# will-rowe/groot

Hardware: AMD Instinct MI355X
Metric: Mreads/s aligned (higher is better)
Workload: dtype u64

## Files before the change

### groot_amd/csrc/hip/device_types.hpp

```cpp
#pragma once

#include <cstdint>

#include <hip/hip_runtime.h>

#include "groot_hip.h"

namespace groot {

constexpr int kBlock = 256;
constexpr uint32_t kEmpty = 0xFFFFFFFFu;

enum : uint32_t {
    kFlagShortRead = 1u,
    kFlagLongRead = 2u,
    kFlagSeedOverflow = 4u,
    kFlagTravOverflow = 8u,
    kFlagOrdOverflow = 16u,
    kFlagOvfOverflow = 32u,
    kFlagQOverflow = 64u,
};

constexpr uint32_t kIncrCap = 8;
constexpr uint32_t kIncrCapBig = 2048;
// ... 167 lines not shown

struct AlignArgs {
    DeviceIndex ix;
    const uint8_t *seq;
    const uint64_t *seq_off;
    uint32_t n_reads, first_read_id;
    uint32_t seed_slots;
    const uint32_t *seed_count;
    const uint32_t *seed_win;
    const uint32_t *perm;
    const ReadRec *read_rec;
    uint32_t no_align, update_weights;
    const void *node_rec;
    uint32_t *attempts;
    groot_trav *trav_first;
    uint64_t *mask_first;
    uint32_t *trav_cnt;
    groot_trav *ovf_trav;
    uint64_t *ovf_mask;
    uint32_t *ovf_cnt;
    uint32_t ovf_cap;
    uint64_t *stk_hdr;
    uint64_t *stk_mask;
    uint32_t n_threads, stk_depth;
    uint32_t lds_stride_dw;
    uint32_t *incr_cnt, *incr_win;
    uint32_t incr_cap;
    uint32_t head_lanes;
    uint32_t round_lanes;
    const uint4 *vitem;
    const uint32_t *vcount;
    uint32_t vcap;
    const uint32_t *n_perm;
    uint32_t refill;
    DeviceCounters *ctr;
};

struct alignas(16) LeanNode {
    uint32_t seq_off;
    uint32_t seq_len;
    uint32_t deg_kids;
    uint32_t pad;
    uint32_t edges[4];
    uint64_t first32;
    uint64_t mask[3];
};
static_assert(sizeof(LeanNode) == 64, "lean node record is one 64-byte line");
constexpr uint32_t kLeanNo = 0x80000000u;
struct alignas(16) LeanExt {
    uint64_t b[7];
    uint64_t pad;
};
static_assert(sizeof(LeanExt) == 64, "lean node extension is one 64-byte line");
constexpr uint32_t kLeanMaxLen = 256;

struct LeanArgs {
    const LeanNode *nodes;
    const LeanExt *ext;
    const uint32_t *bases2;
    const uint4 *cn_pre2;
    const uint64_t *node_l2b;
    const uint8_t *win_ok;
    const WinRec *win_rec;
    const uint32_t *q_row;
    const uint8_t *seq;
    const uint4 *packed;
    uint32_t packed_q;
    const uint32_t *perm;
    const ReadRec *read_rec;
    uint32_t n_reads, first_read_id, n_windows, k;
    uint32_t update_weights;
    uint32_t lds_stride_dw;
    uint32_t max_len;
    uint32_t *attempts;
    groot_trav *trav_first;
    uint64_t *mask_first;
    uint32_t *trav_cnt;
    uint8_t *defer;
    uint4 *stk;
    groot_trav *ovf_trav;
    uint64_t *ovf_mask;
    uint32_t *ovf_cnt;
    uint32_t ovf_cap;
    DeviceCounters *ctr;
    const uint4 *path_node;
    const uint32_t *path_text;
    const uint32_t *path_tag;
    const uint32_t *path_nodes;
    const uint64_t *path_tab;
    uint4 *hold;
};

__host__ __device__ inline uint32_t lean_stride_dw(uint32_t max_len) { return (((max_len + 15u) >> 4) + 15u) | 1u; }

}
```

### groot_amd/csrc/hip/groot_hip.hip

```cpp
#include <cstring>

#include <hip/hip_runtime.h>
#include <rocprim/rocprim.hpp>

#include <dlfcn.h>

#include <algorithm>
#include <cmath>
#include <cstdarg>
#include <cstdio>
#include <atomic>
#include <chrono>
#include <deque>
#include <map>
#include <memory>
#include <numeric>
#include <string>
#include <thread>
#include <vector>

#include "../common/cpus.hpp"
#include "../common/view_check.hpp"
#include "kernels_boot.hpp"
#include "kernels_cov.hpp"
// ... 94 lines not shown
    DevBuf<uint8_t> d_seq, d_exc_byte;
    DevBuf<uint64_t> d_off, d_exc_pos;
    uint32_t trav_cap = 0;
    DevBuf<groot_trav> d_trav;
    DevBuf<uint64_t> d_mask;
    DevBuf<DeviceCounters> d_ctr;
    PinBuf<DeviceCounters> h_ctr;
    PinBuf<groot_trav> h_trav;
    DevBuf<groot_ctrav> d_ctrav;
    PinBuf<groot_ctrav> h_ctrav;
    PinBuf<uint8_t> h_mask;
    PinBuf<uint32_t> h_ckpt;
    DevBuf<uint8_t> d_cmask;
    DevBuf<uint32_t> d_mwords, d_moff, d_ckpt;
    uint32_t n_trav = 0, copied = 0;
    uint64_t n_mask_bytes = 0, copied_bytes = 0;
    bool host_results = false;
    hipEvent_t ev_seed = nullptr;
    hipEvent_t ev_walk = nullptr;
    hipEvent_t ev_h2d0 = nullptr, ev_h2d = nullptr, ev_compute = nullptr, ev_ctr = nullptr, ev_d2h0 = nullptr, ev_d2h = nullptr;
    hipEvent_t ev[14]{};
    groot_counts counts{};
    int status = GROOT_OK;
    std::string status_msg;
    groot_stage_ms ms{};
    DevBuf<uint32_t> d_ec_slow;
    PinBuf<uint32_t> h_ec;
    const uint8_t *seq() const { return input == IN_DEVICE ? ext_seq : d_seq.p; }
    const uint64_t *off() const { return input == IN_DEVICE ? ext_off : d_off.p; }
};

struct WorkSet {
    DevBuf<uint32_t> seed_count, seed_win, perm, perm_count, trav_cnt, tab_idx;
    DevBuf<uint32_t> perm2, perm2_count;
    DevBuf<uint8_t> defer;
    DevBuf<uint4> packed;
    DevBuf<ReadRec> read_rec;
    DevBuf<uint4> vitem, split_list;
    DevBuf<uint32_t> vcount;
    DevBuf<groot_trav> trav_first;
    DevBuf<uint64_t> mask_first, sketches;
    DevBuf<groot_trav> ovf_trav;
    DevBuf<uint64_t> ovf_mask;
    DevBuf<uint32_t> ovf_cnt;
    hipEvent_t ev_free = nullptr;
    bool used = false;
    Slot *owner = nullptr;
    uint64_t ticket = 0;
};

struct groot_ctx {
    int device = 0;
    std::string err;
    groot_params prm{};
    Knobs kn;
    uint32_t s = 0, k = 0, max_k = 0, l_max = 0, pw_view = 0, pw = 0, n_windows = 0, max_q = 0, band_hash_bits = 0;
    hipEvent_t h2d_last = nullptr;
    Slot *newest = nullptr;
    hipEvent_t last_compute = nullptr;
    hipStream_t own_stream = nullptr, stream = nullptr, astream = nullptr, tstream = nullptr, own_tstream = nullptr, h2d_stream = nullptr, d2h_stream = nullptr;
    bool profiling = false;

    DevBuf<uint32_t> graph_win_end;
    DevBuf<uint4> cn_pre;
    DevBuf<uint64_t> node_l2b;
    DevBuf<uint32_t> win_prefix, edges, win_graph, cn_node,
        band_keys, band_ids;
    DevBuf<ExactEntry> band_hash;
// ... 47 lines not shown
    DeviceIndex *build_dix = nullptr;
    hipStream_t build_stream = nullptr;
    unsigned long long *build_shards = nullptr;

    std::vector<std::unique_ptr<Slot>> slots;
    std::deque<Slot *> inflight;
    uint64_t next_ticket = 1;
    Slot *waited = nullptr;
    double todo_frac = 1.0;
    double lean_left_frac = 1.0;
    uint32_t n_cu = 256;
    double dfs_frac = 1.0;
    double trav_per_read = 1.25;
    double bytes_per_trav = 0;
    bool packed_travs = false;
    std::vector<uint32_t> h_node_graph;
    DevBuf<uint8_t> graph_words;
    std::vector<uint8_t> h_graph_words;
    WorkSet ws[2];
    uint32_t next_set = 0;

    uint32_t seed_slots = 0;
    DevBuf<uint32_t> sort_key, sort_key_out, perm_in, todo_list, todo_count;
    DevBuf<uint32_t> long_list, long_count;
    uint32_t vcap = 0;
    uint32_t lsh_defer_rows = 0, lsh_cap = 0;
    DevBuf<unsigned long long> seed_shards;
    DevBuf<uint32_t> lsh_list, lsh_count;
    DevBuf<uint64_t> lsh_sketch;
    DevBuf<char> sort_tmp, in_tmp;
    uint32_t ovf_cap = 0;
    DevBuf<uint32_t> trav_off;
    DevBuf<char> scan_tmp;
    DevBuf<char> sel_tmp;
    uint32_t align_threads = 0, stk_depth = 0;
    DevBuf<uint64_t> stk_hdr, stk_mask;
    DevBuf<uint32_t> attempts, q_row, q_seen, q_of_row, q_nrows;
    uint32_t *attempts_ptr = nullptr;
    uint32_t att_cap = 0;
    bool att_external = false;
    bool cov_on = false;
    std::vector<uint32_t> h_cov_np_off, h_cov_gpo, h_cov_len;
    std::vector<uint2> h_cov_np;
    std::vector<uint64_t> h_cov_base;
    DevBuf<uint32_t> cov_np_off, cov_gpo, cov_len;
    DevBuf<uint2> cov_np;
    DevBuf<uint64_t> cov_base;
    DevBuf<unsigned long long> cov_starts, cov_ends;
    bool sh_on = false;
    uint32_t sh_tab_cap = 0;
    DevBuf<uint32_t> sh_gpo, sh_set_graph, sh_tab_rep, sh_tab_cnt, sh_slow, sh_batch;
    DevBuf<uint64_t> sh_set_mask;
    DevBuf<unsigned long long> sh_tri, sh_stats;
    bool ec_on = false;
    uint32_t ec_cap = 0, ec_epoch = 0;
    DevBuf<uint32_t> ec_claim, ec_graph, ec_fill;
    DevBuf<uint64_t> ec_mask;
    DevBuf<unsigned long long> ec_cnt;
    uint64_t ec_fill_known = 0;
    uint64_t ec_grows = 0, ec_slow_reads = 0;
    std::map<std::vector<uint32_t>, uint64_t> ec_host;
};

__attribute__((constructor)) static void groot_hw_queues() { setenv("GPU_MAX_HW_QUEUES", "8", 0); }

static thread_local std::string g_open_err;

// ... 253 lines not shown
static int grow_attempts(groot_ctx *c, uint32_t rows)
{
    if (c->att_external) return fail(c, GROOT_E_NOSPACE, "a kmerCount outside the fixed layout of groot_hip_attempts_layout occurred");
    DevBuf<uint32_t> bigger;
    HIP_TRY(c, bigger.alloc((size_t)rows * c->n_windows));
    HIP_TRY(c, hipMemset(bigger.p, 0, (size_t)rows * c->n_windows * sizeof(uint32_t)));
    if (c->attempts.p && c->att_cap)
        HIP_TRY(c, hipMemcpy(bigger.p, c->attempts.p, (size_t)std::min(rows, c->att_cap) * c->n_windows * sizeof(uint32_t), hipMemcpyDeviceToDevice));
    std::swap(c->attempts.p, bigger.p);
    std::swap(c->attempts.n, bigger.n);
    c->attempts_ptr = c->attempts.p;
    c->att_cap = rows;
    return GROOT_OK;
}

constexpr double kSparseBelow = 0.05;
struct HasKey {
    const uint32_t *key;
    __host__ __device__ bool operator()(uint32_t r) const { return key[r] != kEmpty; }
};
#ifndef GROOT_SPAN_BITS
#define GROOT_SPAN_BITS 6
#endif
static uint32_t list_lds_stride(uint32_t stride_dw)
{
    return kLdsReads + (uint64_t)kBlock * stride_dw * 4 <= 32 * 1024 ? stride_dw : 0;
}
#ifndef GROOT_HEAVY_BLOCKS
#define GROOT_HEAVY_BLOCKS 16384u
#endif
#ifndef GROOT_SORTLIST_BLOCKS
#define GROOT_SORTLIST_BLOCKS 16384
#endif
static int launch_seed_stage(groot_ctx *c, Slot *s, bool update_weights)
{
    WorkSet *w = &c->ws[s->set];
    SeedArgs a{};
    s->packed_q = 0;
    a.ix = c->dix;
    a.seq = s->seq();
    a.seq_off = s->off();
    a.n_reads = s->n_reads;
    a.max_read_len = c->prm.max_read_len;
    const uint64_t want = (uint64_t)kBlock * s->max_len + 32;
    a.lds_read_bytes = (uint32_t)std::min<uint64_t>(want, kMaxLdsReadBytes);
    a.seed_slots = c->seed_slots;
    a.seed_count = w->seed_count.p;
    a.seed_win = w->seed_win.p;
    a.sketch_out = c->prm.keep_sketches ? w->sketches.p : nullptr;
    a.sort_key = c->sort_key.p;
    a.read_rec = w->read_rec.p;
    a.q_seen = c->q_seen.p;
    a.trav_cnt = w->trav_cnt.p;
    a.shards = c->seed_shards.p;
    a.ctr = s->d_ctr.p;
    a.long_list = c->long_list.p; a.long_count = c->long_count.p;
    if (c->dix.out_tab) {
        a.tab_idx = w->tab_idx.p;
        a.tab_hist = c->tab_hist.p;
    }
    unsigned win_bits = 2;
    for (uint32_t v = c->n_windows ? c->n_windows - 1 : 0; v; v >>= 1) win_bits++;
    win_bits = std::min(32u, std::max(3u, win_bits));
    a.sort_span_bits = std::min((unsigned)GROOT_SPAN_BITS, 32u - win_bits);
    if (win_bits - 2u + a.sort_span_bits > 24u && win_bits - 2u + 4u <= 24u) a.sort_span_bits = 24u - (win_bits - 2u);
    a.sort_span_shift = win_bits;
// ... 58 lines not shown
    HIP_TRY(c, hipGetLastError());
    if (c->profiling) HIP_TRY(c, hipEventRecord(s->ev[12], c->stream));
    {
        SplitArgs sa{};
        sa.list = c->long_list.p; sa.count = c->long_count.p; sa.seed_count = w->seed_count.p; sa.seed_win = w->seed_win.p;
        sa.n_reads = s->n_reads; sa.seed_slots = c->seed_slots; sa.read_rec = w->read_rec.p; sa.win_rec = c->dix.win_rec;
        sa.split = c->vcap && !c->tab_capture && !c->prm.no_exact_align;
        sa.vitem = w->vitem.p; sa.vcount = w->vcount.p; sa.vcap = c->vcap; sa.split_list = w->split_list.p;
        sa.ctr = s->d_ctr.p; sa.update_weights = update_weights ? 1 : 0;
        hipLaunchKernelGGL(sort_seed_lists_kernel, dim3(GROOT_SORTLIST_BLOCKS), dim3(kBlock), 0, c->stream, sa);
    }
    if (c->profiling) HIP_TRY(c, hipEventRecord(s->ev[2], c->stream));
    hipLaunchKernelGGL(assign_q_rows_kernel, dim3(1), dim3(64), 0, c->stream, c->q_seen.p, c->q_row.p, c->q_of_row.p, c->q_nrows.p, c->att_cap,
                       c->max_q, s->d_ctr.p, c->seed_shards.p, c->long_count.p);
    if (a.tab_hist) {
        hipLaunchKernelGGL(fold_tab_hist_kernel, dim3(std::min<uint32_t>((c->n_windows + kBlock - 1) / kBlock, 1024u)), dim3(kBlock), 0, c->stream, c->tab_hist.p,
                           c->attempts_ptr, c->q_row.p, c->dix.w - c->k + 1, c->n_windows, s->d_ctr.p, update_weights ? 1u : 0u);
        HIP_TRY(c, hipGetLastError());
    }
    if (list_mode && a.dfs_list) return GROOT_OK;
    if (list_mode) {
        size_t tb = 0;
        HasKey pred{c->sort_key.p};
        rocprim::counting_iterator<uint32_t> ids(0u);
        HIP_TRY(c, rocprim::select(nullptr, tb, ids, w->perm.p, w->perm_count.p, (size_t)s->n_reads, pred, c->stream));
        if (tb > c->sort_tmp.n) {
            HIP_TRY(c, hipStreamSynchronize(c->stream));
            HIP_TRY(c, c->sort_tmp.alloc(tb + tb / 4));
        }
        HIP_TRY(c, rocprim::select(c->sort_tmp.p, tb, ids, w->perm.p, w->perm_count.p, (size_t)s->n_reads, pred, c->stream));
        return GROOT_OK;
    }
    size_t tmp_bytes = 0;
    HIP_TRY(c, rocprim::radix_sort_pairs(nullptr, tmp_bytes, c->sort_key.p, c->sort_key_out.p, c->perm_in.p, w->perm.p, s->n_reads, begin_bit,
                                         end_bit, c->stream));
    if (tmp_bytes > c->sort_tmp.n) {
        HIP_TRY(c, hipStreamSynchronize(c->stream));
        HIP_TRY(c, c->sort_tmp.alloc(tmp_bytes + tmp_bytes / 4));
    }
    HIP_TRY(c, rocprim::radix_sort_pairs(c->sort_tmp.p, tmp_bytes, c->sort_key.p, c->sort_key_out.p, c->perm_in.p, w->perm.p,
                                         s->n_reads, begin_bit, end_bit, c->stream));
    return GROOT_OK;
}

struct LeanLeft {
    const uint8_t *defer;
    const DeviceCounters *ctr;
    uint32_t lean_slots;
    __device__ uint8_t operator()(uint32_t i) const { return i < ctr->seeded_reads && (i >= lean_slots || defer[i]) ? 1 : 0; }
};

static int launch_align_stage(groot_ctx *c, Slot *s, bool update_weights)
{
    WorkSet *w = &c->ws[s->set];
    AlignArgs a{};
    a.ix = c->dix;
    a.seq = s->seq();
    a.seq_off = s->off();
    a.n_reads = s->n_reads;
    a.first_read_id = s->first_read_id;
    a.seed_slots = c->seed_slots;
    a.seed_count = w->seed_count.p;
    a.seed_win = w->seed_win.p;
    a.perm = w->perm.p;
    a.read_rec = w->read_rec.p;
    a.no_align = c->prm.no_exact_align;
    a.update_weights = update_weights ? 1 : 0;
    a.attempts = c->attempts_ptr;
    a.node_rec = c->node_rec.p;
    a.trav_first = w->trav_first.p;
    a.mask_first = w->mask_first.p;
    a.trav_cnt = w->trav_cnt.p;
    a.ovf_trav = w->ovf_trav.p;
    a.ovf_mask = w->ovf_mask.p;
    a.ovf_cnt = w->ovf_cnt.p;
    a.ovf_cap = c->ovf_cap;
    if (c->vcap) { a.vitem = w->vitem.p; a.vcount = w->vcount.p; a.vcap = c->vcap; }
    a.stk_hdr = c->stk_hdr.p;
    a.stk_mask = c->stk_mask.p;
    uint32_t blocks = std::min<uint32_t>((s->n_reads + kBlock - 1) / kBlock, c->align_threads / kBlock);
    if (c->dfs_frac < kSparseBelow && c->dfs_frac * (double)s->n_reads < 16.0 * (double)(blocks * (kBlock / 64))) blocks = std::max(1u, blocks / 2);
    else if (c->dfs_frac >= kSparseBelow && c->dfs_frac < 0.6 && !s->mixed_len && blocks >= 4) blocks /= 2;
    if ((s->lean_used || s->path_used) && c->lean_left_frac < 0.25) {
        uint32_t want = (uint32_t)(c->lean_left_frac * 1.25 * (double)s->n_reads / 64.0 / (kBlock / 64)) + 1u;
        blocks = std::max(1u, std::min(blocks, std::max(want, c->n_cu)));
    }
    a.n_threads = blocks * kBlock;
    a.stk_depth = c->stk_depth;
    {
        const uint32_t stride = (2 + 4 * ((s->max_len + 27) / 16)) | 1u;
        a.lds_stride_dw = (size_t)kBlock * stride * 4 <= 64 * 1024 ? stride : 0;
    }
    if (c->tab_capture) {
        a.incr_cnt = c->incr_cnt.p; a.incr_win = c->incr_win.p; a.incr_cap = c->incr_cap;
        HIP_TRY(c, hipMemsetAsync(c->incr_cnt.p, 0, (size_t)s->n_reads * sizeof(uint32_t), c->tstream));
    }
    a.head_lanes = s->mixed_len ? 16u : 0u;
#ifndef GROOT_REFILL_ERR
#define GROOT_REFILL_ERR 48
#endif
#ifndef GROOT_REFILL_MIXED
#define GROOT_REFILL_MIXED 2
#endif
    a.refill = s->mixed_len ? (uint32_t)GROOT_REFILL_MIXED : (c->dfs_frac >= kSparseBelow && c->dfs_frac < 0.6 ? (uint32_t)GROOT_REFILL_ERR : 64u);
#ifdef GROOT_WORK_COUNTERS
    if (const char *e = getenv("GROOT_DEV_ROUND")) a.round_lanes = (uint32_t)atoi(e);
#endif
    a.ctr = s->d_ctr.p;
    const bool first_pass = s->lean_used || s->path_used;
    hipStream_t walk = first_pass ? c->astream : c->tstream;
    HIP_TRY(c, hipMemsetAsync(w->ovf_cnt.p, 0, (kOvfShards + 2) * sizeof(uint32_t), walk));
    const uint32_t lean_stride = lean_stride_dw(s->max_len);
    if (first_pass) {
        LeanArgs l{};
        l.nodes = c->lean_nodes.p; l.ext = c->lean_ext.p; l.bases2 = c->bases2.p; l.cn_pre2 = c->cn_pre2.p; l.win_ok = c->win_ok.p;
        l.win_rec = c->dix.win_rec; l.node_l2b = c->dix.node_l2b; l.q_row = c->q_row.p;
        l.seq = s->seq(); l.packed = s->packed_q ? w->packed.p : nullptr; l.packed_q = s->packed_q; l.perm = w->perm.p; l.read_rec = w->read_rec.p;
        l.n_reads = s->n_reads; l.first_read_id = s->first_read_id; l.n_windows = c->n_windows; l.k = c->k;
        l.update_weights = update_weights ? 1 : 0;
        l.lds_stride_dw = lean_stride; l.max_len = s->max_len;
        l.attempts = c->attempts_ptr;
        l.trav_first = w->trav_first.p; l.mask_first = w->mask_first.p; l.trav_cnt = w->trav_cnt.p;
        l.defer = w->defer.p; l.ctr = s->d_ctr.p;
        l.stk = c->lean_stk.p; l.ovf_trav = w->ovf_trav.p; l.ovf_mask = w->ovf_mask.p; l.ovf_cnt = w->ovf_cnt.p; l.ovf_cap = c->ovf_cap;
        const uint32_t lean_blocks = std::min<uint32_t>((s->n_reads + kBlock - 1) / kBlock, (uint32_t)(c->dfs_frac * 1.05 * (double)s->n_reads / kBlock) + 64u);
        if (s->path_used) {
            l.path_node = c->path_node.p; l.path_text = c->path_text.p; l.path_tag = c->path_tag.p; l.path_nodes = c->path_nodes.p; l.path_tab = c->path_tab.p;
            l.hold = c->path_hold.p;
            launch_align_path(c->pw, l, dim3(lean_blocks), c->astream);
        } else launch_align_lean(c->pw, l, dim3(lean_blocks), c->astream);
        HIP_TRY(c, hipGetLastError());
        size_t tb = 0;
        rocprim::counting_iterator<uint32_t> ids(0u);
        auto flags = rocprim::make_transform_iterator(ids, LeanLeft{w->defer.p, s->d_ctr.p, lean_blocks * (uint32_t)kBlock});
        HIP_TRY(c, rocprim::select(nullptr, tb, w->perm.p, flags, w->perm2.p, w->perm2_count.p, (size_t)s->n_reads, c->astream));
        if (tb > c->sel_tmp.n) {
            HIP_TRY(c, hipStreamSynchronize(c->astream));
            HIP_TRY(c, c->sel_tmp.alloc(tb + tb / 4));
        }
        HIP_TRY(c, rocprim::select(c->sel_tmp.p, tb, w->perm.p, flags, w->perm2.p, w->perm2_count.p, (size_t)s->n_reads, c->astream));
        a.perm = w->perm2.p;
        a.n_perm = w->perm2_count.p;
        if (c->profiling) HIP_TRY(c, hipEventRecord(s->ev[13], c->astream));
        if (c->tstream != c->astream) {
            HIP_TRY(c, hipEventRecord(s->ev_walk, c->astream));
            HIP_TRY(c, hipStreamWaitEvent(c->tstream, s->ev_walk, 0));
        }
    }
    launch_align(c->pw, a, dim3(blocks), c->tstream);
    HIP_TRY(c, hipGetLastError());
    return GROOT_OK;
}

static int launch_order_stage(groot_ctx *c, Slot *s, bool update_weights)
{
    WorkSet *w = &c->ws[s->set];
    const uint32_t n = s->n_reads;
    size_t tmp_bytes = 0;
    if (c->vcap) hipLaunchKernelGGL(split_fix_kernel, dim3(256), dim3(kBlock), 0, c->tstream, w->split_list.p, w->vcount.p, w->vitem.p, w->trav_cnt.p, n, s->d_ctr.p,
                                    w->trav_first.p, w->mask_first.p, c->pw, s->first_read_id);
    HIP_TRY(c, rocprim::exclusive_scan(nullptr, tmp_bytes, w->trav_cnt.p, c->trav_off.p, 0u, n, rocprim::plus<uint32_t>(), c->tstream));
    if (tmp_bytes > c->scan_tmp.n) {
        HIP_TRY(c, hipStreamSynchronize(c->tstream));
        HIP_TRY(c, c->scan_tmp.alloc(tmp_bytes + tmp_bytes / 4));
    }
    HIP_TRY(c, rocprim::exclusive_scan(c->scan_tmp.p, tmp_bytes, w->trav_cnt.p, c->trav_off.p, 0u, n, rocprim::plus<uint32_t>(), c->tstream));
    hipLaunchKernelGGL(order_total_kernel, dim3(1), dim3(1), 0, c->tstream, c->trav_off.p, w->trav_cnt.p, n, s->d_ctr.p);
    OrderTabArgs ot{};
    if (c->dix.out_tab) {
        ot.tab_idx = w->tab_idx.p; ot.out_tab = c->dix.out_tab; ot.stride_q = c->dix.out_stride_q; ot.first_read_id = s->first_read_id;
        ot.update_weights = update_weights ? 1 : 0;
        ot.attempts = c->attempts_ptr; ot.q_row = c->q_row.p;
        ot.q_tab = c->dix.w - c->k + 1; ot.n_windows = c->n_windows;
    }
    if (c->profiling) HIP_TRY(c, hipEventRecord(s->ev[9], c->tstream));
// ... 1698 lines not shown
        if (int rc = grow_attempts(c, std::min<uint32_t>(4, c->max_q + 1))) return rc;
    }
    DeviceIndex &x = c->dix;
    x.k = v->kmer_size; x.s = s; x.w = v->window_size; x.num_window_kmers = v->num_window_kmers;
    x.n_windows = n; x.n_nodes = v->n_nodes; x.pw = c->pw;
    x.edges = c->edges.p; x.bases = c->bases.p;
    x.win_prefix = c->win_prefix.p; x.win_graph = c->win_graph.p; x.win_rec = c->win_rec.p; x.cn_node = c->cn_node.p;
    x.win_sketch = c->win_sketch.p; x.exact = c->exact.p; x.band_keys = c->band_keys.p; x.band_ids = c->band_ids.p;
    x.band_hash = c->band_hash.p; x.band_hash_bits = c->band_hash_bits; x.band_sig = c->band_sig.p; x.band_run = c->band_run.p;
    x.max_k = v->max_k; x.l_max = c->l_max; x.q_k = c->q_k.p; x.q_l = c->q_l.p; x.q_min_eq = c->q_min_eq.p; x.max_q = c->max_q;
    x.q_row = c->q_row.p;

    lap("per-kmerCount tables");
    const uint32_t R = c->prm.max_batch_reads;
    HIP_TRY(c, c->sort_key.alloc(R));
    HIP_TRY(c, c->sort_key_out.alloc(R));
    HIP_TRY(c, c->long_list.alloc(kLongListCap));
    HIP_TRY(c, c->long_count.alloc(4));
    HIP_TRY(c, hipMemset(c->long_count.p, 0, 4 * sizeof(uint32_t)));
    {
        std::vector<uint32_t> iota(R);
        std::iota(iota.begin(), iota.end(), 0u);
        HIP_TRY(c, upload(c->perm_in, iota.data(), iota.size()));
    }
    if (int rc = alloc_seed_slots(c, c->prm.max_seeds_per_read)) return rc;
    c->vcap = c->kn.small_buffers ? 8u : std::max<uint32_t>(4096, R / 4);
    for (WorkSet &w : c->ws) {
        HIP_TRY(c, w.seed_count.alloc(R));
        HIP_TRY(c, w.read_rec.alloc(R));
        HIP_TRY(c, w.perm.alloc(R));
        HIP_TRY(c, w.perm_count.alloc(4));
        if (c->lean || c->path) {
            HIP_TRY(c, w.perm2.alloc(R));
            HIP_TRY(c, w.perm2_count.alloc(4));
            HIP_TRY(c, w.defer.alloc(R));
            HIP_TRY(c, w.packed.alloc((size_t)R * (c->prm.max_read_len <= 128 ? 2 : 4)));
        }
        if (c->prm.keep_sketches) HIP_TRY(c, w.sketches.alloc((size_t)R * s));
        HIP_TRY(c, w.trav_first.alloc((size_t)R + c->vcap));
        HIP_TRY(c, w.mask_first.alloc(((size_t)R + c->vcap) * c->pw));
        HIP_TRY(c, w.trav_cnt.alloc((size_t)R + c->vcap));
        HIP_TRY(c, w.vitem.alloc(std::max<uint32_t>(c->vcap, 1)));
        HIP_TRY(c, w.split_list.alloc(kLongListCap));
        HIP_TRY(c, w.vcount.alloc(4));
        HIP_TRY(c, hipMemset(w.vcount.p, 0, 4 * sizeof(uint32_t)));
    }
    HIP_TRY(c, c->trav_off.alloc(R));
    if (c->lean || c->path) HIP_TRY(c, c->lean_stk.alloc((size_t)R * 4));
    if (c->path) HIP_TRY(c, c->path_hold.alloc((size_t)R * 3 * kPathHold));
    for (WorkSet &w : c->ws) HIP_TRY(c, w.ovf_cnt.alloc(kOvfShards + 2));
    if (int rc = alloc_ovf(c, c->kn.small_buffers ? 2u : std::max<uint32_t>(256, R / kOvfShards / 4))) return rc;
    int n_cu = 256;
    (void)hipDeviceGetAttribute(&n_cu, hipDeviceAttributeMultiprocessorCount, c->device);
    c->n_cu = (uint32_t)std::max(n_cu, 1);
    uint32_t per_cu = c->pw > 3 ? kAlignWavesWide : kAlignWaves;
    c->align_threads = std::min<uint32_t>(((R + kBlock - 1) / kBlock) * kBlock, (uint32_t)std::max(n_cu, 1) * per_cu * kBlock);
    c->stk_depth = c->prm.max_read_len;
    HIP_TRY(c, c->stk_hdr.alloc((size_t)c->stk_depth * c->align_threads));
    HIP_TRY(c, c->stk_mask.alloc((size_t)c->stk_depth * c->align_threads * c->pw));
    if (c->l_max <= kLshMaxBands) {
#ifndef GROOT_LSH_DEFER_ROWS
#define GROOT_LSH_DEFER_ROWS 64
#endif
        c->lsh_defer_rows = GROOT_LSH_DEFER_ROWS;
        c->lsh_cap = c->kn.small_buffers ? 4u : std::max<uint32_t>(4096, R / 4);
        HIP_TRY(c, c->lsh_list.alloc(c->lsh_cap));
        HIP_TRY(c, c->lsh_count.alloc(4));
        HIP_TRY(c, c->lsh_sketch.alloc((size_t)c->lsh_cap * s));
    }
    HIP_TRY(c, c->todo_list.alloc(R));
    HIP_TRY(c, c->todo_count.alloc(1));
    HIP_TRY(c, c->seed_shards.alloc((size_t)kSeedShards * kSeedShardStride));
    HIP_TRY(c, hipMemset(c->seed_shards.p, 0, (size_t)kSeedShards * kSeedShardStride * sizeof(unsigned long long)));
    HIP_TRY(c, hipDeviceSynchronize());
    lap("work buffers");
    c->build_shards = c->seed_shards.p;
    const uint32_t q_w = v->window_size >= v->kmer_size ? v->window_size - v->kmer_size + 1 : 0;
    const bool w_exact = q_w && q_w < c->h_q_min_eq.size() && c->h_q_min_eq[q_w] == s;
    const bool memo_wanted = !c->kn.no_outcome_table && c->prm.memo_budget_mb != GROOT_MEMO_OFF && !c->prm.no_exact_align && !c->prm.keep_sketches;
    if ((flags & GROOT_OPEN_BACKGROUND) && !memo_wanted) {
        if (int rc = finish_lsh()) return rc;
        lap("LSH forest tables (waited for)");
        c->bg_dix = c->dix;
// ... 1195 lines not shown
```

### groot_amd/csrc/hip/kernels_align.hpp

```cpp
#pragma once

#include "kernels_common.hpp"

namespace groot {


enum : uint32_t { PH_FETCH, PH_SCAN, PH_DFS, PH_WAIT, PH_DONE, PH_FORK, PH_FORKWAIT, PH_JOIN };
#ifndef GROOT_FORK_MIN
#define GROOT_FORK_MIN 3
#endif
constexpr uint32_t kForkMin = GROOT_FORK_MIN;
constexpr uint32_t kClsHelper = 0x1000u;
constexpr uint32_t kCoopMin = 6;
constexpr uint32_t kCoopWant = 0xFFFFFFFEu;
#ifndef GROOT_COOP_MAX_ASK
#define GROOT_COOP_MAX_ASK 8
#endif
constexpr uint32_t kCoopMaxAsk = GROOT_COOP_MAX_ASK;
#ifndef GROOT_TL_LATE_US
#define GROOT_TL_LATE_US 3000
#endif
#ifndef GROOT_WAVE_CHUNK
#define GROOT_WAVE_CHUNK 128
#endif
// ... 30 lines not shown
};

template <int PW, bool LDSR>
__global__ __launch_bounds__(kBlock, PW > 3 ? kAlignWavesWide : kAlignWaves) void align_kernel(AlignArgs a)
{
    using Rec = NodeRec<PW>;
    extern __shared__ __attribute__((aligned(16))) uint32_t lds_reads[];
    __shared__ unsigned long long red[4];
    uint32_t *my_lds = lds_reads + (size_t)threadIdx.x * a.lds_stride_dw;
    const DeviceIndex &ix = a.ix;
    const Rec *recs = reinterpret_cast<const Rec *>(a.node_rec);
    const uint32_t gtid = blockIdx.x * kBlock + threadIdx.x;
    if (a.ctr->flags & (kFlagSeedOverflow | kFlagQOverflow)) return;
#ifndef GROOT_ALIGN_PRIO
#define GROOT_ALIGN_PRIO 3
#endif
#if GROOT_ALIGN_PRIO >= 0
    __builtin_amdgcn_s_setprio(GROOT_ALIGN_PRIO);
#endif
    unsigned long long alns = 0, mapped = 0, multimapped = 0, panics = 0;
#ifdef GROOT_WORK_COUNTERS
    uint32_t ev = 0;
    uint32_t wc_iter = 0, wc_round0 = 0;
    unsigned long long wc_t[3] = {0, 0, 0};
    uint32_t wc_n[3] = {0, 0, 0};
    uint32_t wc_n0[3] = {0, 0, 0};
#define GROOT_EV(i) (ev |= 1u << (i))
#else
#define GROOT_EV(i) ((void)0)
#endif

    uint32_t phase = PH_WAIT;
    const uint32_t nv = a.vitem ? min((uint32_t)__builtin_amdgcn_readfirstlane((int)*a.vcount), a.vcap) : 0u;
    const uint32_t n_todo = nv + (a.perm ? min(a.n_reads, (uint32_t)__builtin_amdgcn_readfirstlane((int)(a.n_perm ? *a.n_perm : a.ctr->seeded_reads))) : a.n_reads);
#ifndef GROOT_MIXED_ROUND_LANES
#define GROOT_MIXED_ROUND_LANES 32
#endif
    uint32_t U = a.head_lanes ? (uint32_t)GROOT_MIXED_ROUND_LANES : 64u;
    if (a.round_lanes) U = a.round_lanes;
    else
        while (U > 1u && n_todo < U * (gridDim.x * (uint32_t)(kBlock / 64))) U >>= 1;
    const uint32_t n_rounds = (n_todo + U - 1u) / U;
    const uint32_t head_rounds = (n_rounds >> 3) | 1u;
    const uint32_t Uh = a.head_lanes ? min(a.head_lanes, U) : U;
    const uint32_t head_slots = min(head_rounds * U, n_todo);
    const uint32_t head_small = (head_slots + Uh - 1u) / Uh;
    uint32_t chunk_len = 0, chunk_base = 0;
    bool head_done = head_small == 0;
    const uint32_t chunk_rounds = a.head_lanes ? 1u : kWaveChunk / 64u;
    auto take_chunk = [&]() {
        uint32_t c = 0, tail = 0;
        if ((threadIdx.x & 63) == 0) {
            if (!head_done) c = atomicAdd(a.ovf_cnt + kOvfShards, 1u);
            if (head_done || c >= head_small) {
                tail = 1;
                c = atomicAdd(a.ovf_cnt + kOvfShards + 1, chunk_rounds);
            }
        }
        c = (uint32_t)__builtin_amdgcn_readfirstlane((int)c);
        tail = (uint32_t)__builtin_amdgcn_readfirstlane((int)tail);
        if (tail) {
            head_done = true;
            const unsigned long long b = (unsigned long long)head_slots + (unsigned long long)c * U;
            chunk_base = b > 0xFFFFFFFFull ? 0xFFFFFFFFu : (uint32_t)b;
            chunk_len = chunk_rounds * U;
        } else {
            chunk_base = c * Uh;
// ... 270 lines not shown
        const int cf = __popcll(bf), cs = __popcll(bs), cd = __popcll(bd);
        const uint32_t run = (cd >= cs && cd >= cf) ? PH_DFS : (cs >= cf ? PH_SCAN : PH_FETCH);
        if (phase != run) continue;
        GROOT_EV(run);
#ifdef GROOT_WORK_COUNTERS
        const unsigned long long wc_t0 = wall_clock64();
        const uint32_t wc_steps0 = wc_iter;
#endif
        bool advance = false;

        if (run == PH_FETCH) {
#if defined(GROOT_WORK_COUNTERS) && GROOT_WORK_COUNTERS == 2
#define GROOT_SUBT(i) do { const unsigned long long t__ = wall_clock64(); if ((threadIdx.x & 63) == (__ffsll((unsigned long long)__ballot(1)) - 1)) atomicAdd(&a.ctr->dbg[40 + (i)], t__ - wc_sub); wc_sub = t__; } while (0)
            unsigned long long wc_sub = wall_clock64();
#else
#define GROOT_SUBT(i) ((void)0)
#endif
            if (!have_read) {
                GROOT_EV(3);
#if defined(GROOT_WORK_COUNTERS) && GROOT_WORK_COUNTERS == 2
                wc_n0[0] = wc_n[0]; wc_n0[1] = wc_n[1]; wc_n0[2] = wc_n[2];
#endif
#if defined(GROOT_WORK_COUNTERS) && GROOT_WORK_COUNTERS == 3
                tl_read0 = wall_clock64(); tl_it0 = wc_iter; tl_st0 = wc_n[0] + wc_n[1] + wc_n[2];
#endif
                const bool virt = slot < nv;
                uint32_t vlo = 0, vhi = 0;
                if (virt) {
                    const uint4 vi = a.vitem[slot];
                    r = vi.x; vlo = vi.y; vhi = vi.z;
                    if (r == kEmpty) { phase = PH_WAIT; continue; }
                } else {
                    const uint32_t so = slot - nv;
                    r = a.perm ? a.perm[so] : so;
                }
                uint4 ra, rb;
                load32(a.read_rec + r, ra, rb);
                const uint32_t sc = ra.w;
                cnt = min(sc & (kRecSplit - 1u), a.seed_slots);
                cls = a.perm ? (sc >> 24) & 0x3Fu : 0x80u;
                if (sc & kRecAscending) cls |= 0x100u;
                if (sc & kRecSplit) cls |= 0xA00u;
                if (virt) { cnt = min(vhi, a.seed_slots); cls = 0x80u | 0x100u | 0x200u | 0x400u; }
                if (cnt == 0) { a.trav_cnt[r] = 0; phase = PH_WAIT; continue; }
                high_byte = sc >> 31;
                len = ra.z & ~kRecPacked;
                p = a.seq + ((uint64_t)ra.x | ((uint64_t)ra.y << 32));
                sd0 = rb.x; sd1 = rb.y; sd2 = rb.z; sd3 = rb.w;
                if (cls & 0x200u) sd0 = vlo;
                else if (cnt > 4 && (cls & 0x100u)) sd0 = 0;
                GROOT_SUBT(0);
                if (LDSR && 2 + 4 * ((len + 27) >> 4) > a.lds_stride_dw) {
                    atomicOr(&a.ctr->flags, kFlagLongRead);
                    a.trav_cnt[(cls & 0x400u) ? a.n_reads + slot : r] = 0;
                    phase = PH_WAIT;
                    continue;
                }
                qrow = ix.q_row[len - ix.k + 1];
                read_id = a.first_read_id + ((cls & 0x400u) ? a.n_reads + slot : r);
                n_graphs = 0; ord = 0; last = -1; fk = 0;
                done_graph = kEmpty; cur_graph = kEmpty; group_rc_called = false;
                have_read = true;
                if (LDSR) {
                    my_lds[0] = 0; my_lds[1] = 0;
                    for (uint32_t b = 0; b < len; b += 64) {
                        const uint4 *src = reinterpret_cast<const uint4 *>(p + b);
                        const bool h1 = b + 16 < len, h2 = b + 32 < len, h3 = b + 48 < len;
// ... 422 lines not shown
```

### groot_amd/csrc/hip/kernels_lean.hpp

```cpp
#pragma once

#include "kernels_common.hpp"
#include "kernels_path.hpp"

namespace groot {


#ifndef GROOT_LEAN_WAVES
#define GROOT_LEAN_WAVES 5
#endif
constexpr int kLeanWaves = GROOT_LEAN_WAVES;
#ifndef GROOT_LEAN_MAX_ITER
#define GROOT_LEAN_MAX_ITER 96
#endif
constexpr uint32_t kLeanMaxIter = GROOT_LEAN_MAX_ITER;

__device__ __forceinline__ uint64_t lean_lowmask(int n) { return n <= 0 ? 0ull : (n >= 32 ? ~0ull : ((1ull << (2 * n)) - 1ull)); }
__device__ __forceinline__ uint32_t lean_revcomp16(uint32_t v)
{
    uint32_t r = __brev(v);
    r = ((r & 0xAAAAAAAAu) >> 1) | ((r & 0x55555555u) << 1);
    return r ^ 0xAAAAAAAAu;
}
__device__ __forceinline__ uint64_t lean_funnel(uint32_t x0, uint32_t x1, uint32_t x2, uint32_t sh)
// ... 434 lines not shown
                    const uint4 h0 = stk[2 * sp], h1 = stk[2 * sp + 1];
                    cur = h0.x & 0x7FFFFFFFu; cur_long = h0.x >> 31; coff = 0; dist = h0.y;
                    m0 = (uint64_t)h0.z | ((uint64_t)h0.w << 32);
                    m1 = (uint64_t)h1.x | ((uint64_t)h1.y << 32);
                    m2 = (uint64_t)h1.z | ((uint64_t)h1.w << 32);
                    cur64 = chunk(dist);
                } else if (emitted) { done_graph = g; st = ST_SEED; }
                else st = pos >= lim ? ST_ADV : ST_GEN;
            }
        }
    }

#if defined(GROOT_WORK_COUNTERS) && GROOT_WORK_COUNTERS == 4
    if ((threadIdx.x & 63) == 0) {
        const unsigned long long t2 = wall_clock64();
        for (int i = 0; i < 9; i++) atomicAdd(&a.ctr->dbg[140 + i], lw[i]);
        atomicAdd(&a.ctr->dbg[149], lw_t1 - lw_t0);
        atomicAdd(&a.ctr->dbg[150], t2 - lw_t1);
        atomicAdd(&a.ctr->dbg[151], 1ull);
    }
    for (uint32_t y = 1; y <= 10; y++) {
        const unsigned long long b = __ballot(st == ST_DEFER && why == y);
        if (b && (threadIdx.x & 63) == 0) atomicAdd(&a.ctr->dbg[160 + y], (unsigned long long)__popcll(b));
    }
    { const unsigned long long b = __ballot(st == ST_DONE && !ord); if (b && (threadIdx.x & 63) == 0) atomicAdd(&a.ctr->dbg[160], (unsigned long long)__popcll(b)); }
    for (uint32_t y = 11; y <= 13; y++) {
        const unsigned long long b = __ballot(st == ST_DEFER && why == y);
        if (b && (threadIdx.x & 63) == 0) atomicAdd(&a.ctr->dbg[160 + y], (unsigned long long)__popcll(b));
    }
    if (PATH)
        for (int i = 0; i < 5; i++) if (stops[i]) atomicAdd(&a.ctr->dbg[176 + i], (unsigned long long)stops[i]);
#endif
    const bool fin = st == ST_DONE;
    if (slot < n_todo) a.defer[slot] = st == ST_DEFER ? 1 : 0;
    unsigned long long n_alns = 0, mapped = 0, multimapped = 0;
    if (fin) {
        a.trav_cnt[r] = ord;
        if (PATH)
            for (uint32_t o = 1; o < ord; o++) {
                const uint4 h0 = hold[3 * (o - 1)], h1 = hold[3 * (o - 1) + 1], h2 = hold[3 * (o - 1) + 2];
                groot_trav t_;
                t_.read_id = a.first_read_id + r; t_.graph_id = h0.x; t_.node = h0.y; t_.offset = h0.z;
                t_.ord = (uint16_t)(h0.w & 0xFFFFu); t_.flags = (uint8_t)(h0.w >> 16); t_.reserved = 0;
                const uint32_t shard = blockIdx.x & (kOvfShards - 1);
                const uint32_t at = atomicAdd(&a.ovf_cnt[shard], 1u);
                if (at < a.ovf_cap) {
                    const size_t q = (size_t)shard * a.ovf_cap + at;
                    a.ovf_trav[q] = t_;
                    a.ovf_mask[q * PW] = (uint64_t)h1.x | ((uint64_t)h1.y << 32);
                    a.ovf_mask[q * PW + 1] = (uint64_t)h1.z | ((uint64_t)h1.w << 32);
                    a.ovf_mask[q * PW + 2] = (uint64_t)h2.x | ((uint64_t)h2.y << 32);
                } else atomicOr(&a.ctr->flags, kFlagOvfOverflow);
            }
        mapped = 1;
        multimapped = n_graphs > 1u ? 1 : 0;
        n_alns = alns;
    }
    if (a.update_weights) {
        const uint32_t qrow = fin ? a.q_row[len - a.k + 1u] : 0u;
        const uint64_t cell = (uint64_t)qrow * a.n_windows + (fin ? W[W_WIN] : 0u);
        const unsigned long long here = __ballot(fin);
        const unsigned lane_ = threadIdx.x & 63u;
        const unsigned long long below = here & ((1ull << lane_) - 1ull);
        const int prev = below ? 63 - __builtin_clzll(below) : -1;
        const uint32_t plo = __shfl((uint32_t)cell, prev < 0 ? (int)lane_ : prev), phi = __shfl((uint32_t)(cell >> 32), prev < 0 ? (int)lane_ : prev);
        const bool head = fin && (prev < 0 || plo != (uint32_t)cell || phi != (uint32_t)(cell >> 32));
        const unsigned long long heads = __ballot(head);
// ... 30 lines not shown
```

Measured before the change: 2280.

## Emit deferred reads via wave-aggregated atomics and tune order radix sort config

The lean/path kernel no longer writes a per-slot defer byte that a later rocprim::select pass compacts. Instead each wave appends its deferred read ids to a list using one ballot-aggregated atomic. The align kernel reads that list first, then walks the untouched tail of the permutation beyond the lean slots directly, so the select launch and its temp buffer are gone. Separately, the order radix sort uses a custom onesweep config with 256-thread blocks, except on error batches. Deferred reads now land in nondeterministic order, and the tail handling adds indexing logic to the align kernel.

```diff
diff --git a/groot_amd/csrc/hip/device_types.hpp b/groot_amd/csrc/hip/device_types.hpp
--- a/groot_amd/csrc/hip/device_types.hpp
+++ b/groot_amd/csrc/hip/device_types.hpp
@@ -223,6 +223,8 @@
     const uint32_t *vcount;
     uint32_t vcap;
     const uint32_t *n_perm;
+    const uint32_t *rest;
+    uint32_t rest_lo;
     uint32_t refill;
     DeviceCounters *ctr;
 };
@@ -267,7 +269,8 @@
     groot_trav *trav_first;
     uint64_t *mask_first;
     uint32_t *trav_cnt;
-    uint8_t *defer;
+    uint32_t *left;
+    uint32_t *left_cnt;
     uint4 *stk;
     groot_trav *ovf_trav;
     uint64_t *ovf_mask;
diff --git a/groot_amd/csrc/hip/groot_hip.hip b/groot_amd/csrc/hip/groot_hip.hip
--- a/groot_amd/csrc/hip/groot_hip.hip
+++ b/groot_amd/csrc/hip/groot_hip.hip
@@ -150,8 +150,7 @@
 
 struct WorkSet {
     DevBuf<uint32_t> seed_count, seed_win, perm, perm_count, trav_cnt, tab_idx;
-    DevBuf<uint32_t> perm2, perm2_count;
-    DevBuf<uint8_t> defer;
+    DevBuf<uint32_t> perm2;
     DevBuf<uint4> packed;
     DevBuf<ReadRec> read_rec;
     DevBuf<uint4> vitem, split_list;
@@ -265,7 +264,6 @@
     uint32_t ovf_cap = 0;
     DevBuf<uint32_t> trav_off;
     DevBuf<char> scan_tmp;
-    DevBuf<char> sel_tmp;
     uint32_t align_threads = 0, stk_depth = 0;
     DevBuf<uint64_t> stk_hdr, stk_mask;
     DevBuf<uint32_t> attempts, q_row, q_seen, q_of_row, q_nrows;
@@ -585,6 +583,20 @@
 #ifndef GROOT_SORTLIST_BLOCKS
 #define GROOT_SORTLIST_BLOCKS 16384
 #endif
+#ifndef GROOT_SORT_ITEMS
+#define GROOT_SORT_ITEMS 16
+#endif
+#ifndef GROOT_SORT_MERGE_LIMIT
+#define GROOT_SORT_MERGE_LIMIT 2048
+#endif
+using OrderSortConfig = rocprim::radix_sort_config<
+    rocprim::default_config, rocprim::default_config,
+    rocprim::radix_sort_onesweep_config<rocprim::kernel_config<256, GROOT_SORT_ITEMS>, rocprim::kernel_config<256, GROOT_SORT_ITEMS>, 8,
+                                        rocprim::block_radix_rank_algorithm::match>,
+    GROOT_SORT_MERGE_LIMIT>;
+
+static bool error_batch(const groot_ctx *c, const Slot *s) { return c->dfs_frac >= kSparseBelow && c->dfs_frac < 0.6 && !s->mixed_len; }
+
 static int launch_seed_stage(groot_ctx *c, Slot *s, bool update_weights)
 {
     WorkSet *w = &c->ws[s->set];
@@ -709,23 +721,21 @@
         return GROOT_OK;
     }
     size_t tmp_bytes = 0;
-    HIP_TRY(c, rocprim::radix_sort_pairs(nullptr, tmp_bytes, c->sort_key.p, c->sort_key_out.p, c->perm_in.p, w->perm.p, s->n_reads, begin_bit,
-                                         end_bit, c->stream));
+    const bool small_blocks = !error_batch(c, s);
+    auto sort = [&](void *tmp) {
+        return small_blocks ? rocprim::radix_sort_pairs<OrderSortConfig>(tmp, tmp_bytes, c->sort_key.p, c->sort_key_out.p, c->perm_in.p, w->perm.p, s->n_reads,
+                                                                         begin_bit, end_bit, c->stream)
+                            : rocprim::radix_sort_pairs(tmp, tmp_bytes, c->sort_key.p, c->sort_key_out.p, c->perm_in.p, w->perm.p, s->n_reads, begin_bit, end_bit,
+                                                        c->stream);
+    };
+    HIP_TRY(c, sort(nullptr));
     if (tmp_bytes > c->sort_tmp.n) {
         HIP_TRY(c, hipStreamSynchronize(c->stream));
         HIP_TRY(c, c->sort_tmp.alloc(tmp_bytes + tmp_bytes / 4));
     }
-    HIP_TRY(c, rocprim::radix_sort_pairs(c->sort_tmp.p, tmp_bytes, c->sort_key.p, c->sort_key_out.p, c->perm_in.p, w->perm.p,
-                                         s->n_reads, begin_bit, end_bit, c->stream));
-    return GROOT_OK;
-}
-
-struct LeanLeft {
-    const uint8_t *defer;
-    const DeviceCounters *ctr;
-    uint32_t lean_slots;
-    __device__ uint8_t operator()(uint32_t i) const { return i < ctr->seeded_reads && (i >= lean_slots || defer[i]) ? 1 : 0; }
-};
+    HIP_TRY(c, sort(c->sort_tmp.p));
+    return GROOT_OK;
+}
 
 static int launch_align_stage(groot_ctx *c, Slot *s, bool update_weights)
 {
@@ -757,7 +767,7 @@
     a.stk_mask = c->stk_mask.p;
     uint32_t blocks = std::min<uint32_t>((s->n_reads + kBlock - 1) / kBlock, c->align_threads / kBlock);
     if (c->dfs_frac < kSparseBelow && c->dfs_frac * (double)s->n_reads < 16.0 * (double)(blocks * (kBlock / 64))) blocks = std::max(1u, blocks / 2);
-    else if (c->dfs_frac >= kSparseBelow && c->dfs_frac < 0.6 && !s->mixed_len && blocks >= 4) blocks /= 2;
+    else if (error_batch(c, s) && blocks >= 4) blocks /= 2;
     if ((s->lean_used || s->path_used) && c->lean_left_frac < 0.25) {
         uint32_t want = (uint32_t)(c->lean_left_frac * 1.25 * (double)s->n_reads / 64.0 / (kBlock / 64)) + 1u;
         blocks = std::max(1u, std::min(blocks, std::max(want, c->n_cu)));
@@ -779,14 +789,14 @@
 #ifndef GROOT_REFILL_MIXED
 #define GROOT_REFILL_MIXED 2
 #endif
-    a.refill = s->mixed_len ? (uint32_t)GROOT_REFILL_MIXED : (c->dfs_frac >= kSparseBelow && c->dfs_frac < 0.6 ? (uint32_t)GROOT_REFILL_ERR : 64u);
+    a.refill = s->mixed_len ? (uint32_t)GROOT_REFILL_MIXED : (error_batch(c, s) ? (uint32_t)GROOT_REFILL_ERR : 64u);
 #ifdef GROOT_WORK_COUNTERS
     if (const char *e = getenv("GROOT_DEV_ROUND")) a.round_lanes = (uint32_t)atoi(e);
 #endif
     a.ctr = s->d_ctr.p;
     const bool first_pass = s->lean_used || s->path_used;
     hipStream_t walk = first_pass ? c->astream : c->tstream;
-    HIP_TRY(c, hipMemsetAsync(w->ovf_cnt.p, 0, (kOvfShards + 2) * sizeof(uint32_t), walk));
+    HIP_TRY(c, hipMemsetAsync(w->ovf_cnt.p, 0, (kOvfShards + 3) * sizeof(uint32_t), walk));
     const uint32_t lean_stride = lean_stride_dw(s->max_len);
     if (first_pass) {
         LeanArgs l{};
@@ -798,7 +808,7 @@
         l.lds_stride_dw = lean_stride; l.max_len = s->max_len;
         l.attempts = c->attempts_ptr;
         l.trav_first = w->trav_first.p; l.mask_first = w->mask_first.p; l.trav_cnt = w->trav_cnt.p;
-        l.defer = w->defer.p; l.ctr = s->d_ctr.p;
+        l.left = w->perm2.p; l.left_cnt = w->ovf_cnt.p + kOvfShards + 2; l.ctr = s->d_ctr.p;
         l.stk = c->lean_stk.p; l.ovf_trav = w->ovf_trav.p; l.ovf_mask = w->ovf_mask.p; l.ovf_cnt = w->ovf_cnt.p; l.ovf_cap = c->ovf_cap;
         const uint32_t lean_blocks = std::min<uint32_t>((s->n_reads + kBlock - 1) / kBlock, (uint32_t)(c->dfs_frac * 1.05 * (double)s->n_reads / kBlock) + 64u);
         if (s->path_used) {
@@ -807,17 +817,10 @@
             launch_align_path(c->pw, l, dim3(lean_blocks), c->astream);
         } else launch_align_lean(c->pw, l, dim3(lean_blocks), c->astream);
         HIP_TRY(c, hipGetLastError());
-        size_t tb = 0;
-        rocprim::counting_iterator<uint32_t> ids(0u);
-        auto flags = rocprim::make_transform_iterator(ids, LeanLeft{w->defer.p, s->d_ctr.p, lean_blocks * (uint32_t)kBlock});
-        HIP_TRY(c, rocprim::select(nullptr, tb, w->perm.p, flags, w->perm2.p, w->perm2_count.p, (size_t)s->n_reads, c->astream));
-        if (tb > c->sel_tmp.n) {
-            HIP_TRY(c, hipStreamSynchronize(c->astream));
-            HIP_TRY(c, c->sel_tmp.alloc(tb + tb / 4));
-        }
-        HIP_TRY(c, rocprim::select(c->sel_tmp.p, tb, w->perm.p, flags, w->perm2.p, w->perm2_count.p, (size_t)s->n_reads, c->astream));
         a.perm = w->perm2.p;
-        a.n_perm = w->perm2_count.p;
+        a.n_perm = l.left_cnt;
+        a.rest = w->perm.p;
+        a.rest_lo = lean_blocks * (uint32_t)kBlock;
         if (c->profiling) HIP_TRY(c, hipEventRecord(s->ev[13], c->astream));
         if (c->tstream != c->astream) {
             HIP_TRY(c, hipEventRecord(s->ev_walk, c->astream));
@@ -2582,8 +2585,6 @@
         HIP_TRY(c, w.perm_count.alloc(4));
         if (c->lean || c->path) {
             HIP_TRY(c, w.perm2.alloc(R));
-            HIP_TRY(c, w.perm2_count.alloc(4));
-            HIP_TRY(c, w.defer.alloc(R));
             HIP_TRY(c, w.packed.alloc((size_t)R * (c->prm.max_read_len <= 128 ? 2 : 4)));
         }
         if (c->prm.keep_sketches) HIP_TRY(c, w.sketches.alloc((size_t)R * s));
@@ -2598,7 +2599,7 @@
     HIP_TRY(c, c->trav_off.alloc(R));
     if (c->lean || c->path) HIP_TRY(c, c->lean_stk.alloc((size_t)R * 4));
     if (c->path) HIP_TRY(c, c->path_hold.alloc((size_t)R * 3 * kPathHold));
-    for (WorkSet &w : c->ws) HIP_TRY(c, w.ovf_cnt.alloc(kOvfShards + 2));
+    for (WorkSet &w : c->ws) HIP_TRY(c, w.ovf_cnt.alloc(kOvfShards + 3));
     if (int rc = alloc_ovf(c, c->kn.small_buffers ? 2u : std::max<uint32_t>(256, R / kOvfShards / 4))) return rc;
     int n_cu = 256;
     (void)hipDeviceGetAttribute(&n_cu, hipDeviceAttributeMultiprocessorCount, c->device);
diff --git a/groot_amd/csrc/hip/kernels_align.hpp b/groot_amd/csrc/hip/kernels_align.hpp
--- a/groot_amd/csrc/hip/kernels_align.hpp
+++ b/groot_amd/csrc/hip/kernels_align.hpp
@@ -86,7 +86,10 @@
 
     uint32_t phase = PH_WAIT;
     const uint32_t nv = a.vitem ? min((uint32_t)__builtin_amdgcn_readfirstlane((int)*a.vcount), a.vcap) : 0u;
-    const uint32_t n_todo = nv + (a.perm ? min(a.n_reads, (uint32_t)__builtin_amdgcn_readfirstlane((int)(a.n_perm ? *a.n_perm : a.ctr->seeded_reads))) : a.n_reads);
+    const uint32_t n_seeded = min(a.n_reads, (uint32_t)__builtin_amdgcn_readfirstlane((int)a.ctr->seeded_reads));
+    const uint32_t n_list = a.n_perm ? min(a.n_reads, (uint32_t)__builtin_amdgcn_readfirstlane((int)*a.n_perm)) : n_seeded;
+    const uint32_t n_rest = a.rest && n_seeded > a.rest_lo ? n_seeded - a.rest_lo : 0u;
+    const uint32_t n_todo = nv + (a.perm ? min(a.n_reads, n_list + n_rest) : a.n_reads);
 #ifndef GROOT_MIXED_ROUND_LANES
 #define GROOT_MIXED_ROUND_LANES 32
 #endif
@@ -423,7 +426,7 @@
                     if (r == kEmpty) { phase = PH_WAIT; continue; }
                 } else {
                     const uint32_t so = slot - nv;
-                    r = a.perm ? a.perm[so] : so;
+                    r = !a.perm ? so : so < n_list ? a.perm[so] : a.rest[a.rest_lo + (so - n_list)];
                 }
                 uint4 ra, rb;
                 load32(a.read_rec + r, ra, rb);
diff --git a/groot_amd/csrc/hip/kernels_lean.hpp b/groot_amd/csrc/hip/kernels_lean.hpp
--- a/groot_amd/csrc/hip/kernels_lean.hpp
+++ b/groot_amd/csrc/hip/kernels_lean.hpp
@@ -490,7 +490,18 @@
         for (int i = 0; i < 5; i++) if (stops[i]) atomicAdd(&a.ctr->dbg[176 + i], (unsigned long long)stops[i]);
 #endif
     const bool fin = st == ST_DONE;
-    if (slot < n_todo) a.defer[slot] = st == ST_DEFER ? 1 : 0;
+    {
+        const bool left = st == ST_DEFER && slot < n_todo;
+        const unsigned long long lb = __ballot(left);
+        if (lb) {
+            const unsigned lane_ = threadIdx.x & 63u;
+            const int first = __ffsll(lb) - 1;
+            uint32_t at = 0;
+            if ((int)lane_ == first) at = atomicAdd(a.left_cnt, (uint32_t)__popcll(lb));
+            at = __shfl(at, first);
+            if (left) a.left[at + (uint32_t)__popcll(lb & ((1ull << lane_) - 1ull))] = r;
+        }
+    }
     unsigned long long n_alns = 0, mapped = 0, multimapped = 0;
     if (fin) {
         a.trav_cnt[r] = ord;
```

Measured after the change: 2347, median of 6. 2.9% higher.
